# arancormonk/mbelib-neo

Measured on AMD Instinct MI355X. Metric: 20ms frames/sec (whole node) + PCM RMS error vs reference, IMBE 7200x4400, higher is better.
Workload: dtype f32

## Files before the change

mbelib-neo_amd/csrc/mbx_expand_imbe.h:

```cpp
#pragma once
#include "mbx_device.h"
#include "mbx_expand_ambe.h"
#ifndef MBX_FTS
#define MBX_FTS(i, v) do { } while (0)
#endif

namespace mbx {
namespace xp {

__device__ __forceinline__ uint32_t low_bits_x(uint32_t v, int n) { return v & ((1u << n) - 1u); }

__device__ __forceinline__ void expand_imbe_frame_rec(bool have, uint4 rec, float* row, uint32_t* words, float* gains, int sub,
                                                      const DeviceTables& tabs) {
    const mbx_tables* T = tabs.t;
    {
        uint4* z = reinterpret_cast<uint4*>(&words[8 * sub]);
        z[0] = make_uint4(0u, 0u, 0u, 0u);
        z[1] = make_uint4(0u, 0u, 0u, 0u);
    }
    int bad = 1, L = 0, K = 0;
    float w0 = 0.0f;
    if (have) {
        const uint32_t w[3] = {rec.x, rec.y, rec.z};
        int b0 = (int)(w[0] >> 26);
        b0 = (b0 << 1) | rbit(w, 85);
        b0 = (b0 << 1) | rbit(w, 86);
        if (b0 <= 207) {
            const uint2 q = tabs.d->imbe_b0[b0];
            w0 = __uint_as_float(q.x);
            L = (int)(q.y & 0xffu);
            K = (int)(q.y >> 8);
            bad = (L == 0) ? 1 : 0;
        }
    } else {
        rec = make_uint4(0u, 0u, 0u, 0u);
    }
    MBX_FTS(5, L);
    const int L9 = bad ? 0 : L - 9;
    const bool live = have && !bad;
    const bool block_lane = live && sub >= 1 && sub <= 6;
    const DerivedTables* D = tabs.d;
    uint32_t e[10];
    {
        const uint16_t* bo = reinterpret_cast<const uint16_t*>(&T->imbe_bo[L9][0][0]);
#pragma unroll
        for (int t = 0; t < 10; ++t) {
            const int idx = 10 * sub + t;
            e[t] = bo[idx < 79 ? idx : 78];
        }
    }
    const int blk = block_lane ? sub : 1;
    const uint32_t info = D->imbe_blk_info[L9][blk];
    const int g = (sub >= 2 && sub <= 6) ? sub - 2 : 0;
    const float nb = T->imbe_ba[L9][g][0], step = T->imbe_ba[L9][g][1];
    float ric[7];
#pragma unroll
    for (int m = 1; m <= 6; ++m) {
        ric[m] = T->imbe_ri_cos[m][blk];
    }
    float qstep[11];
    uint32_t bmw[3];
    {
        const uint32_t* bp = reinterpret_cast<const uint32_t*>(&D->imbe_blk_bm[L9][blk][0]);
        bmw[0] = bp[0];
        bmw[1] = bp[1];
        bmw[2] = bp[2];
#pragma unroll
        for (int k = 2; k <= 10; ++k) {
            qstep[k] = D->imbe_blk_step[L9][blk][k];
        }
    }
    const int ji_rows = (int)((info >> 16) & 0xffu);
    const float* rows = &D->imbe_len_rows[ji_rows <= 10 ? ji_rows : 10][0][0];
    float cosr[10];
#pragma unroll
    for (int k = 0; k < 10; ++k) {
        cosr[k] = rows[k];
    }
    MBX_FTS(6, cosr[0]);
    wave_lds_sync();
    {
        const int s0 = 10 * sub + 6;
        const uint32_t hi = s0 < 32 ? rec.x : (s0 < 64 ? rec.y : rec.z), lo = s0 < 32 ? rec.y : (s0 < 64 ? rec.z : 0u);
        uint32_t window = (uint32_t)(((((uint64_t)hi << 32) | lo) << (s0 & 31)) >> 54);
        window &= (sub == 7) ? ~1u : ~0u;
#pragma unroll
        for (int t = 0; t < 10; ++t) {
            const uint32_t m = e[t] & 0xffu, pos = e[t] >> 8;
            atomicOr(&words[m], ((window >> (9 - t)) & 1u) << pos);
        }
    }
    wave_lds_sync();
    MBX_FTS(7, e[0]);
    float b2v = 0.0f;
    if (live && sub == 1) {
        b2v = T->imbe_B2[low_bits_x(words[2], 6)];
    }
    if (block_lane) {
        float G = b2v;
        if (sub != 1) {
            const int inb = (int)nb;
            const int bm = (int)low_bits_x(words[sub + 1], inb);
            G = (step * ((float)bm - ldexpf(1.0f, inb - 1) + 0.5f));
        }
        gains[sub] = G;
    }
    wave_lds_sync();
    MBX_FTS(8, b2v);
    const uint32_t b1 = low_bits_x(words[1], 12);
    uint32_t band_lo = 0u, band_hi = 0u;
#pragma unroll
    for (int h = 0; h < 2; ++h) {
        const int k = sub + 8 * h;
        if (k < 12 && k < K && ((b1 >> (K - 1 - k)) & 1u)) {
            const unsigned long long m = 7ULL << (3 * k);
            band_lo |= (uint32_t)m;
            band_hi |= (uint32_t)(m >> 32);
        }
    }
    band_lo = sum8(band_lo);
    band_hi = sum8(band_hi);
    if (have) {
        if (sub == 0) {
            uint32_t vlo = 0, vhi = 0;
            if (!bad) {
                unsigned long long v = ((unsigned long long)band_hi << 32) | band_lo;
                if (b1 & 1u) {
                    v |= ~0ULL << (3 * K);
                }
                v &= (L >= 64) ? ~0ULL : ((1ULL << L) - 1ULL);
                vlo = (uint32_t)v;
                vhi = (uint32_t)(v >> 32);
            }
            row[0] = 0.0f;
            row[57] = __uint_as_float(vlo);
            row[58] = __uint_as_float(vhi);
            row[59] = w0;
            row[60] = __int_as_float(L);
            row[61] = __int_as_float(K);
            row[62] = __uint_as_float(rec.w);
            row[63] = __int_as_float(bad);
        } else if (block_lane) {
            const int m0 = (int)(info & 0xffu), l0 = (int)((info >> 8) & 0xffu), ji = (int)((info >> 16) & 0xffu);
            float C2[11];
            {
                float sum = 0;
#pragma unroll
                for (int m = 1; m <= 6; ++m) {
                    const float am = (m == 1) ? 1.0f : 2.0f;
                    sum = sum + (am * gains[m] * ric[m]);
                }
                C2[1] = sum;
            }
#pragma unroll
            for (int k = 2; k <= 10; ++k) {
                const int Bm = (int)((bmw[k >> 2] >> (8 * (k & 3))) & 0xffu);
                const int bm = (int)low_bits_x(words[m0 + k - 2], Bm);
                const float v = (qstep[k] * (((float)bm - ldexpf(1.0f, Bm - 1)) + 0.5f));
                C2[k] = 2.0f * v;
            }
            float next[10];
            auto fetch = [&](float (&dst)[10], int j) {
                const float* nr = rows + 10 * (j < ji ? j : ji - 1);
#pragma unroll
                for (int k = 0; k < 10; ++k) {
                    dst[k] = nr[k];
                }
            };
            auto output = [&](const float (&c)[10], int j) {
                float sum = 0;
#pragma unroll
                for (int k = 1; k <= 10; ++k) {
                    sum = sum + (C2[k] * c[k - 1]);
                }
                row[l0 + j - 1] = sum;
            };
            for (int j = 1; j <= ji; j += 2) {
                fetch(next, j);
                output(cosr, j);
                if (j + 1 <= ji) {
                    fetch(cosr, j + 1);
                    output(next, j + 1);
                }
            }
        }
    }
}

}
}
```

mbelib-neo_amd/csrc/mbx_stream.hip:

```cpp
#include <type_traits>

#include "mbx_device.h"
#include "mbx_kernels.h"
#include "mbx_expand_ambe.h"
#ifdef MBX_STAGE_TIMES
namespace mbx {
constexpr int kStageWaves = 65536;
__device__ unsigned g_stage_buf[kStageWaves * 16];
__shared__ unsigned long long s_stage_prev;
}
#define MBX_TS(i)                                                                          \
    do {                                                                                   \
        const unsigned long long t_ = wall_clock64();                                      \
        if ((threadIdx.x & 63) == 0) {                                                     \
            if ((i) > 0 && blockIdx.x < (unsigned)mbx::kStageWaves) {                      \
                mbx::g_stage_buf[blockIdx.x * 16u + (unsigned)(i)] = (unsigned)(t_ - mbx::s_stage_prev);   \
            }                                                                              \
            mbx::s_stage_prev = t_;                                                        \
        }                                                                                  \
    } while (0)
#else
#define MBX_TS(i) do { } while (0)
#endif
#if defined(MBX_STAGE_TIMES) && defined(MBX_STAGE_SUB)
#define MBX_TSX(i) MBX_TS(i)
#else
#define MBX_TSX(i) do { } while (0)
#endif
#ifdef MBX_FRAME_STAMPS
namespace mbx { __device__ unsigned long long g_frame_stamps[16]; }
#define MBX_FSTAMP(i) do { g_frame_stamps[i] = wall_clock64(); } while (0)
#endif
#ifdef MBX_STAGE_TIMES
#define MBX_FTS(i, v) do { asm volatile("" :: "v"(v)); MBX_TS(i); } while (0)
#else
#define MBX_FTS(i, v) do { } while (0)
#endif
#include "mbx_fec_frame.h"
#include "mbx_front_imbe.h"

#ifndef MBX_PRIO_BANK
#define MBX_PRIO_BANK 2
#endif
#ifndef MBX_PRIO_FFT
#define MBX_PRIO_FFT 1
#endif
#ifndef MBX_PRIO_FRONT_IMBE
#define MBX_PRIO_FRONT_IMBE 3
#endif
#ifndef MBX_PRIO_FRONT_BLOCK
#define MBX_PRIO_FRONT_BLOCK 3
#endif
#ifndef MBX_PARK_N
#define MBX_PARK_N 8
#endif
#ifndef MBX_STREAM_WAVES_PER_SIMD
#define MBX_STREAM_WAVES_PER_SIMD 7
#endif

namespace mbx {

struct Parms {
    float    w0;
    int      L, K;
    int      Vl;
    float    Ml, log2Ml, PHIl, PSIl;
    float    gamma;
    uint32_t tonePhase;
    int      swn;
    float    localEnergy;
    int      amplitudeThreshold;
    float    errorRate;
    int      errorCountTotal, errorCount4, repeatCount;
    float    mutingThreshold;
    float    uw[4];
    float    noiseSeed;
    float    ov[2];
};

__device__ __forceinline__ float uni(float x) { return __int_as_float(__builtin_amdgcn_readfirstlane(__float_as_int(x))); }
__device__ __forceinline__ int uni(int x) { return __builtin_amdgcn_readfirstlane(x); }
__device__ __forceinline__ uint32_t uni(uint32_t x) { return (uint32_t)__builtin_amdgcn_readfirstlane((int)x); }

enum : int {
    O_W0 = 0, O_L = 1, O_K = 2, O_VL = 3, O_ML = 60, O_LOG2ML = 117, O_PHI = 174, O_PSI = 231, O_GAMMA = 288,
    O_TONEPHASE = 289, O_SWN = 290, O_LOCALENERGY = 291, O_AMPTHR = 292, O_ERRORRATE = 293, O_ERRTOTAL = 294,
    O_ERR4 = 295, O_REPEAT = 296, O_MUTETHR = 297, O_UW = 298, O_NOISESEED = 554, O_OVERLAP = 555, PARMS_DWORDS = 651
};

enum : int {
    H_W0 = 0, H_L = 1, H_K = 2, H_GAMMA = 3, H_TONEPHASE = 4, H_SWN = 5, H_LOCALENERGY = 6, H_AMPTHR = 7, H_ERRORRATE = 8,
    H_ERRTOTAL = 9, H_ERR4 = 10, H_REPEAT = 11, H_MUTETHR = 12, H_NOISESEED = 13
};
__device__ __forceinline__ uint32_t load_header(const mbe_parms* __restrict__ p, int lane) {
    const int j = lane & 15;
    const int idx = (j < 3) ? j : ((j < 13) ? (O_GAMMA - H_GAMMA) + j : O_NOISESEED);
    static_assert(O_MUTETHR - O_GAMMA == H_MUTETHR - H_GAMMA, "fields 3..12 of the header are contiguous in mbe_parms");
    return reinterpret_cast<const uint32_t*>(p)[idx];
}
__device__ __forceinline__ int hdr_i(uint32_t h, int k) { return __builtin_amdgcn_readlane((int)h, k); }
__device__ __forceinline__ float hdr_f(uint32_t h, int k) { return __int_as_float(__builtin_amdgcn_readlane((int)h, k)); }

template <bool kFlat = false>
__device__ __forceinline__ void load_parms_arrays(Parms& r, const mbe_parms* __restrict__ p, int lane) {
    const float* f = reinterpret_cast<const float*>(p);
    const int* i = reinterpret_cast<const int*>(p);
    const bool band = lane < MBX_BAND_SLOTS;
    if constexpr (kFlat) {
        const int vl = i[O_VL + lane];
        const float ml = f[O_ML + lane], l2 = f[O_LOG2ML + lane], ph = f[O_PHI + lane], ps = f[O_PSI + lane];
#pragma unroll
        for (int j = 0; j < 4; ++j) {
            r.uw[j] = f[O_UW + lane + 64 * j];
        }
        r.ov[0] = f[O_OVERLAP + lane];
        const float o1 = f[O_OVERLAP + 64 + (lane & 31)];
        r.Vl = band ? vl : 0;
        r.Ml = band ? ml : 0.0f;
        r.log2Ml = band ? l2 : 0.0f;
        r.PHIl = band ? ph : 0.0f;
        r.PSIl = band ? ps : 0.0f;
        r.ov[1] = (lane < 32) ? o1 : 0.0f;
        return;
    }
    r.Vl = band ? i[O_VL + lane] : 0;
    r.Ml = band ? f[O_ML + lane] : 0.0f;
    r.log2Ml = band ? f[O_LOG2ML + lane] : 0.0f;
    r.PHIl = band ? f[O_PHI + lane] : 0.0f;
    r.PSIl = band ? f[O_PSI + lane] : 0.0f;
#pragma unroll
    for (int j = 0; j < 4; ++j) {
        r.uw[j] = f[O_UW + lane + 64 * j];
    }
    r.ov[0] = f[O_OVERLAP + lane];
    r.ov[1] = (lane < 32) ? f[O_OVERLAP + 64 + lane] : 0.0f;
}
__device__ __forceinline__ void set_parms_header(Parms& r, uint32_t h) {
    r.w0 = hdr_f(h, H_W0);
    r.L = hdr_i(h, H_L);
    r.K = hdr_i(h, H_K);
    r.gamma = hdr_f(h, H_GAMMA);
    r.tonePhase = (uint32_t)hdr_i(h, H_TONEPHASE);
    r.swn = hdr_i(h, H_SWN);
    r.localEnergy = hdr_f(h, H_LOCALENERGY);
    r.amplitudeThreshold = hdr_i(h, H_AMPTHR);
    r.errorRate = hdr_f(h, H_ERRORRATE);
    r.errorCountTotal = hdr_i(h, H_ERRTOTAL);
    r.errorCount4 = hdr_i(h, H_ERR4);
    r.repeatCount = hdr_i(h, H_REPEAT);
    r.mutingThreshold = hdr_f(h, H_MUTETHR);
    r.noiseSeed = hdr_f(h, H_NOISESEED);
}
template <bool kGather = false>
__device__ __forceinline__ void load_parms(Parms& r, const mbe_parms* __restrict__ p, int lane) {
    if constexpr (kGather) {
        const uint32_t h = load_header(p, lane);
        load_parms_arrays(r, p, lane);
        set_parms_header(r, h);
        return;
    }
    const float* f = reinterpret_cast<const float*>(p);
    const int* i = reinterpret_cast<const int*>(p);
    r.w0 = uni(f[O_W0]);
    r.L = uni(i[O_L]);
    r.K = uni(i[O_K]);
    load_parms_arrays(r, p, lane);
    r.gamma = uni(f[O_GAMMA]);
    r.tonePhase = (uint32_t)uni(i[O_TONEPHASE]);
    r.swn = uni(i[O_SWN]);
    r.localEnergy = uni(f[O_LOCALENERGY]);
    r.amplitudeThreshold = uni(i[O_AMPTHR]);
    r.errorRate = uni(f[O_ERRORRATE]);
    r.errorCountTotal = uni(i[O_ERRTOTAL]);
    r.errorCount4 = uni(i[O_ERR4]);
    r.repeatCount = uni(i[O_REPEAT]);
    r.mutingThreshold = uni(f[O_MUTETHR]);
    r.noiseSeed = uni(f[O_NOISESEED]);
}

__device__ __forceinline__ int write_lane(int v, int uniform_value, int k) {
    asm("v_writelane_b32 %0, %1, %2" : "+v"(v) : "s"(__builtin_amdgcn_readfirstlane(uniform_value)), "n"(k));
    return v;
}
template <bool kNt, class T>
__device__ __forceinline__ void st_state(T* p, T v) {
    if constexpr (kNt) {
        __builtin_nontemporal_store(v, p);
    } else {
        *p = v;
    }
}
enum UwSkip : int { kUwStoreAll = 0, kUwSkipUpper = 1, kUwSkipAll = 2 };
__device__ __forceinline__ bool uw_all_zero_bits(float a, float b, float c = 0.0f, float d = 0.0f) {
    const uint32_t bits = (__float_as_uint(a) | __float_as_uint(b)) | (__float_as_uint(c) | __float_as_uint(d));
    return __ballot(bits != 0u) == 0ULL;
}
template <bool kGather = false, bool kNt = kGather, bool kSilent = false>
__device__ __forceinline__ void store_parms(const Parms& r, mbe_parms* __restrict__ p, int lane, UwSkip uw_skip = kUwStoreAll) {
    float* f = reinterpret_cast<float*>(p);
    int* i = reinterpret_cast<int*>(p);
    if constexpr (kGather) {
        int h = 0;
        h = write_lane(h, __float_as_int(r.w0), H_W0);
        h = write_lane(h, r.L, H_L);
        h = write_lane(h, r.K, H_K);
        h = write_lane(h, __float_as_int(r.gamma), H_GAMMA);
        h = write_lane(h, (int)r.tonePhase, H_TONEPHASE);
        h = write_lane(h, r.swn, H_SWN);
        h = write_lane(h, __float_as_int(r.localEnergy), H_LOCALENERGY);
        h = write_lane(h, r.amplitudeThreshold, H_AMPTHR);
        h = write_lane(h, __float_as_int(r.errorRate), H_ERRORRATE);
        h = write_lane(h, r.errorCountTotal, H_ERRTOTAL);
        h = write_lane(h, r.errorCount4, H_ERR4);
        h = write_lane(h, r.repeatCount, H_REPEAT);
        h = write_lane(h, __float_as_int(r.mutingThreshold), H_MUTETHR);
        h = write_lane(h, __float_as_int(r.noiseSeed), H_NOISESEED);
        if (lane < 14) {
            const int idx = (lane < 3) ? lane : ((lane < 13) ? (O_GAMMA - H_GAMMA) + lane : O_NOISESEED);
            st_state<kNt>(&i[idx], (int)(h));
        }
    } else if (lane == 0) {
        st_state<kNt>(&f[O_W0], (float)(r.w0));
        st_state<kNt>(&i[O_L], (int)(r.L));
        st_state<kNt>(&i[O_K], (int)(r.K));
        st_state<kNt>(&f[O_GAMMA], (float)(r.gamma));
        st_state<kNt>(&i[O_TONEPHASE], (int)((int)r.tonePhase));
        st_state<kNt>(&i[O_SWN], (int)(r.swn));
        st_state<kNt>(&f[O_LOCALENERGY], (float)(r.localEnergy));
        st_state<kNt>(&i[O_AMPTHR], (int)(r.amplitudeThreshold));
        st_state<kNt>(&f[O_ERRORRATE], (float)(r.errorRate));
        st_state<kNt>(&i[O_ERRTOTAL], (int)(r.errorCountTotal));
        st_state<kNt>(&i[O_ERR4], (int)(r.errorCount4));
        st_state<kNt>(&i[O_REPEAT], (int)(r.repeatCount));
        st_state<kNt>(&f[O_MUTETHR], (float)(r.mutingThreshold));
        st_state<kNt>(&f[O_NOISESEED], (float)(r.noiseSeed));
    }
    if (lane < MBX_BAND_SLOTS) {
        st_state<kNt>(&i[O_VL + lane], (int)(r.Vl));
        st_state<kNt>(&f[O_ML + lane], (float)(r.Ml));
        st_state<kNt>(&f[O_LOG2ML + lane], (float)(r.log2Ml));
        st_state<kNt>(&f[O_PHI + lane], (float)(r.PHIl));
        st_state<kNt>(&f[O_PSI + lane], (float)(r.PSIl));
    }
    if constexpr (kSilent) {
        if (uw_skip != kUwSkipAll) {
            st_state<kNt>(&f[O_UW + lane], (float)(r.uw[0]));
            st_state<kNt>(&f[O_UW + lane + 64], (float)(r.uw[1]));
        }
        if (uw_skip == kUwStoreAll) {
            st_state<kNt>(&f[O_UW + lane + 128], (float)(r.uw[2]));
            st_state<kNt>(&f[O_UW + lane + 192], (float)(r.uw[3]));
        }
    } else {
#pragma unroll
        for (int j = 0; j < 4; ++j) {
            st_state<kNt>(&f[O_UW + lane + 64 * j], (float)(r.uw[j]));
        }
    }
    st_state<kNt>(&f[O_OVERLAP + lane], (float)(r.ov[0]));
    if (lane < 32) {
        st_state<kNt>(&f[O_OVERLAP + 64 + lane], (float)(r.ov[1]));
    }
}

template <bool kFlat = false>
__device__ __forceinline__ void load_prev_arrays(Parms& r, const mbe_parms* __restrict__ p, int lane) {
    const float* f = reinterpret_cast<const float*>(p);
    const bool band = lane < MBX_BAND_SLOTS;
    r = Parms{};
    if constexpr (kFlat) {
        const float ml = f[O_ML + lane], l2 = f[O_LOG2ML + lane], ph = f[O_PHI + lane];
        r.Ml = band ? ml : 0.0f;
        r.log2Ml = band ? l2 : 0.0f;
        r.PHIl = band ? ph : 0.0f;
        return;
    }
    r.Ml = band ? f[O_ML + lane] : 0.0f;
    r.log2Ml = band ? f[O_LOG2ML + lane] : 0.0f;
    r.PHIl = band ? f[O_PHI + lane] : 0.0f;
}
__device__ __forceinline__ void set_prev_header(Parms& r, uint32_t h) {
    r.L = hdr_i(h, H_L);
    r.gamma = hdr_f(h, H_GAMMA);
    r.errorRate = hdr_f(h, H_ERRORRATE);
    r.repeatCount = hdr_i(h, H_REPEAT);
    r.mutingThreshold = hdr_f(h, H_MUTETHR);
}
__device__ __forceinline__ void load_prev_view(Parms& r, const mbe_parms* __restrict__ p, int lane) {
    const uint32_t h = load_header(p, lane);
    load_prev_arrays(r, p, lane);
    set_prev_header(r, h);
}

__device__ __forceinline__ void load_prev_view_lds(Parms& r, const mbe_parms* __restrict__ p, int lane) {
    const float* f = reinterpret_cast<const float*>(p);
    const int* i = reinterpret_cast<const int*>(p);
    load_prev_arrays(r, p, lane);
    r.L = uni(i[O_L]);
    r.gamma = uni(f[O_GAMMA]);
    r.errorRate = uni(f[O_ERRORRATE]);
    r.repeatCount = uni(i[O_REPEAT]);
    r.mutingThreshold = uni(f[O_MUTETHR]);
}

template <bool kFlat = false>
__device__ __forceinline__ void load_enh_arrays(Parms& r, const mbe_parms* __restrict__ p, int lane) {
    const float* f = reinterpret_cast<const float*>(p);
    const int* i = reinterpret_cast<const int*>(p);
    const bool band = lane < MBX_BAND_SLOTS;
    r = Parms{};
    if constexpr (kFlat) {
        const int vl = i[O_VL + lane];
        const float ml = f[O_ML + lane], ph = f[O_PHI + lane], ps = f[O_PSI + lane];
        r.uw[2] = f[O_UW + lane + 128];
        r.uw[3] = f[O_UW + lane + 192];
        r.Vl = band ? vl : 0;
        r.Ml = band ? ml : 0.0f;
        r.PHIl = band ? ph : 0.0f;
        r.PSIl = band ? ps : 0.0f;
        return;
    }
    r.Vl = band ? i[O_VL + lane] : 0;
    r.Ml = band ? f[O_ML + lane] : 0.0f;
    r.PHIl = band ? f[O_PHI + lane] : 0.0f;
    r.PSIl = band ? f[O_PSI + lane] : 0.0f;
    r.uw[2] = f[O_UW + lane + 128];
    r.uw[3] = f[O_UW + lane + 192];
}
__device__ __forceinline__ void set_enh_header(Parms& r, uint32_t h) {
    r.w0 = hdr_f(h, H_W0);
    r.L = hdr_i(h, H_L);
    r.localEnergy = hdr_f(h, H_LOCALENERGY);
    r.amplitudeThreshold = hdr_i(h, H_AMPTHR);
}
__device__ __forceinline__ void load_enh_view(Parms& r, const mbe_parms* __restrict__ p, int lane) {
    const uint32_t h = load_header(p, lane);
    load_enh_arrays(r, p, lane);
    set_enh_header(r, h);
}

__device__ __forceinline__ void prev_header_of(Parms& r, const Parms& cur) {
    r.L = cur.L;
    r.gamma = cur.gamma;
    r.errorRate = cur.errorRate;
    r.repeatCount = cur.repeatCount;
    r.mutingThreshold = cur.mutingThreshold;
}
__device__ __forceinline__ void enh_view_of(Parms& r, const Parms& cur) {
    r = Parms{};
    r.Vl = cur.Vl;
    r.Ml = cur.Ml;
    r.PHIl = cur.PHIl;
    r.PSIl = cur.PSIl;
    r.uw[2] = cur.uw[2];
    r.uw[3] = cur.uw[3];
}

__device__ __forceinline__ void load_continuity(Parms& r, const mbe_parms* __restrict__ p, int lane) {
    const float* f = reinterpret_cast<const float*>(p);
    const bool band = lane < MBX_BAND_SLOTS;
    r.PHIl = band ? f[O_PHI + lane] : 0.0f;
    r.PSIl = band ? f[O_PSI + lane] : 0.0f;
#pragma unroll
    for (int j = 0; j < 4; ++j) {
        r.uw[j] = f[O_UW + lane + 64 * j];
    }
    r.noiseSeed = uni(f[O_NOISESEED]);
    r.ov[0] = f[O_OVERLAP + lane];
    r.ov[1] = (lane < 32) ? f[O_OVERLAP + 64 + lane] : 0.0f;
}

typedef float v2f __attribute__((ext_vector_type(2)));
__device__ __forceinline__ v2f splat(float x) { return v2f{x, x}; }

template <int kParkColsT>
struct WaveScratchT {
    static constexpr int kParkCols = kParkColsT;
    union {
        struct {
            alignas(16) float4 coef_amp[64];
            alignas(16) float4 coef_drift[64];
            alignas(16) float4 icoef[8];
        };
        struct {
            uint32_t words[64];
            float    gains[12];
            float    C[84];
            float    fp[64];
        } x;
        struct {
            float2 fft[256];
            float  bins[144];
        };
    };
    float park[kParkColsT > 0 ? kParkColsT : 1][kParkColsT > 0 ? 64 : 4];
};
using WaveScratch = WaveScratchT<MBX_PARK_N>;

constexpr uint32_t lcg_mul_steps(int n) {
    uint64_t a = 1;
    for (int k = 0; k < n; ++k) {
        a = (a * 171u) % 53125u;
    }
    return (uint32_t)a;
}
constexpr uint32_t lcg_add_steps(int n) {
    uint64_t c = 0;
    for (int k = 0; k < n; ++k) {
        c = (c * 171u + 11213u) % 53125u;
    }
    return (uint32_t)c;
}
constexpr int kDppWaveShr1 = 0x138;
__device__ __forceinline__ float seq_sum4(float v, int L, float* , int ) {
    float acc = v;
    const int n = uni(L);
    auto step = [&]() {
        const float below = __int_as_float(__builtin_amdgcn_update_dpp(0, __float_as_int(acc), kDppWaveShr1, 0xf, 0xf, true));
        acc = below + v;
    };
    int t = n - 1;
    for (; t >= 4; t -= 4) {
        step();
        step();
        step();
        step();
    }
    for (; t > 0; --t) {
        step();
    }
    return __int_as_float(__builtin_amdgcn_readlane(__float_as_int(acc), n & 63));
}

struct StreamRng {
    unsigned long long cn_seed48;
    uint32_t           cn_seeded, unv_state, unv_override;
};

typedef const __attribute__((address_space(4))) mbx_tables* ConstTables;
typedef const __attribute__((address_space(4))) DerivedTables* ConstDerived;
#define MBX_GLOBAL __attribute__((address_space(1)))
typedef const MBX_GLOBAL mbx_tables* GlobalTables;
typedef const MBX_GLOBAL DerivedTables* GlobalDerived;
typedef const MBX_GLOBAL float* GlobalFloats;
__device__ __forceinline__ uint32_t low_bits(uint32_t v, int n) { return v & ((1u << n) - 1u); }

template <class T>
__device__ __forceinline__ T tab_at(const void* uniform_base, size_t uniform_bytes, uint32_t lane_bytes) {
    const MBX_GLOBAL char* p = (const MBX_GLOBAL char*)uniform_base + uniform_bytes;
    asm("" : "+s"(p));
    return *(const MBX_GLOBAL T*)(p + lane_bytes);
}

__device__ __forceinline__ uint4 load_record_scalar(const mbx_param_record* rp) {
    const __attribute__((address_space(4))) uint32_t* rq = (const __attribute__((address_space(4))) uint32_t*)rp;
    return make_uint4(rq[0], rq[1], rq[2], rq[3]);
}

struct ImbeExpandReq {
    int      bad, L;
    uint32_t w0_bits, lk;
    uint32_t e0, e1, own;
    v2f      bas;
    float    b2, qs, sd;
    int      Bm;
// ... 417 lines not shown

__device__ __forceinline__ unsigned long long java_lcg_jump(unsigned long long s, int k) {
    const unsigned long long mask = (1ULL << 48) - 1ULL;
    unsigned long long A = 1, C = 0, a = 0x5DEECE66DULL, c = 0xBULL;
    for (int bit = 0; bit < 8; ++bit) {
        if ((k >> bit) & 1) {
            C = (a * C + c) & mask;
            A = (A * a) & mask;
        }
        c = (a * c + c) & mask;
        a = (a * a) & mask;
    }
    return (A * s + C) & mask;
}

__device__ void comfort_noise(float out[3], StreamRng& rng, int lane) {
    if (!rng.cn_seeded) {
        rng.cn_seed48 = (0x12345678ULL ^ 0x5DEECE66DULL) & ((1ULL << 48) - 1ULL);
        rng.cn_seeded = 1;
    }
    const float gain = (0.003f * 32767.0f) / 7.0f;
#pragma unroll
    for (int j = 0; j < 3; ++j) {
        const int n = lane + 64 * j;
        const unsigned long long s = java_lcg_jump(rng.cn_seed48, n + 1);
        const float u = ((float)(uint32_t)(s >> 24) / 16777216.0f) * 2.0f - 1.0f;
        out[j] = u * gain;
    }
    rng.cn_seed48 = java_lcg_jump(rng.cn_seed48, 160);
}

__device__ __forceinline__ v2f cmul_pk(v2f u, v2f w) {
    v2f t, d;
    asm("v_pk_mul_f32 %0, %1, %2 op_sel_hi:[0,1]" : "=v"(t) : "v"(u), "v"(w));
    asm("v_pk_fma_f32 %0, %1, %2, %3 op_sel:[1,1,0] op_sel_hi:[1,0,1] neg_lo:[0,1,0]" : "=v"(d) : "v"(u), "v"(w), "v"(t));
    return d;
}
__device__ __forceinline__ v2f cmul_cw(v2f u, v2f w) {
    v2f t, d;
    asm("v_pk_mul_f32 %0, %1, %2 op_sel_hi:[0,1] neg_hi:[0,1]" : "=v"(t) : "v"(u), "v"(w));
    asm("v_pk_fma_f32 %0, %1, %2, %3 op_sel:[1,1,0] op_sel_hi:[1,0,1]" : "=v"(d) : "v"(u), "v"(w), "v"(t));
    return d;
}
__device__ __forceinline__ v2f cmul_cu(v2f u, v2f w) {
    v2f t, d;
    asm("v_pk_mul_f32 %0, %1, %2 op_sel_hi:[0,1]" : "=v"(t) : "v"(u), "v"(w));
    asm("v_pk_fma_f32 %0, %1, %2, %3 op_sel:[1,1,0] op_sel_hi:[1,0,1] neg_hi:[0,1,0]" : "=v"(d) : "v"(u), "v"(w), "v"(t));
    return d;
}
__device__ __forceinline__ v2f add_mi(v2f a, v2f b) {
    v2f d;
    asm("v_pk_add_f32 %0, %1, %2 op_sel:[0,1] op_sel_hi:[1,0] neg_hi:[0,1]" : "=v"(d) : "v"(a), "v"(b));
    return d;
}
__device__ __forceinline__ v2f sub_mi(v2f a, v2f b) {
    v2f d;
    asm("v_pk_add_f32 %0, %1, %2 op_sel:[0,1] op_sel_hi:[1,0] neg_lo:[0,1]" : "=v"(d) : "v"(a), "v"(b));
    return d;
}

__device__ __forceinline__ float wrap_two_pi(float x, bool active) {
    const float y = 2.0f * (float)M_PI;
    if (__ballot(active && !(x >= 0.0f && x < 4.0e6f)) != 0ULL) {
        float w = fmodf(x, y);
        if (w < 0.0f) {
            w += y;
        }
        return w;
    }
    const float n = truncf(x * (0.15915494f * 1.000001f));
    float r = fmaf(-n, y, x);
    if (r < 0.0f) {
        r += y;
    }
    return r;
}

__device__ __forceinline__ float div_by_uniform(float a, float b, float rcp_b) {
    const float q = a * rcp_b;
    const float r = fmaf(-q, b, a);
    return fmaf(r, rcp_b, q);
}

template <bool kSnap, bool kPark = false, class Scratch = WaveScratch, bool kEarly = false, bool kDriftUnrolled = false>
__device__ bool synth_core(float out[3], Parms& cur, Parms& prev, bool have_rm0, float rm0, StreamRng& rng,
                           Scratch& S, const DeviceTables& tabs, int lane, const mbe_parms* snap_ptr = nullptr) {
    constexpr int kParkN = Scratch::kParkCols;
    if (kSnap && !kPark) {
        asm volatile("" : "+s"(snap_ptr));
    }
    const mbe_parms* const snap = kSnap ? snap_ptr : nullptr;
    auto snap_f = [&](int dword) -> float {
        if constexpr (kPark) {
            return reinterpret_cast<const float*>(snap)[dword];
        } else {
            return ((GlobalFloats)snap)[dword];
        }
    };
    GlobalDerived D = (GlobalDerived)tabs.d;
    constexpr int N = 160;
    out[0] = out[1] = out[2] = 0.0f;
    __builtin_amdgcn_s_setprio(0);
    if (cur.L < 1 || cur.L > 56 || prev.L < 1 || prev.L > 56) {
        return false;
    }
    if (!have_rm0) {
        const bool in = lane >= 1 && lane <= cur.L;
        rm0 = seq_sum4(in ? (cur.Ml * cur.Ml) : 0.0f, cur.L, reinterpret_cast<float*>(S.fft), lane);
    }
    smooth(cur, prev, rm0, lane, (kSnap && have_rm0) ? reinterpret_cast<const float*>(snap) + O_ML : nullptr,
           reinterpret_cast<float*>(S.fft));

    const bool rate_mutes = fabsf(cur.mutingThreshold - MBE_MUTING_THRESHOLD_AMBE) > 1e-6f;
    if (cur.repeatCount >= MBE_MAX_FRAME_REPEATS || (rate_mutes && cur.errorRate > cur.mutingThreshold)) {
        comfort_noise(out, rng, lane);
        return false;
    }

    float nz[4];
    const bool cold = cur.noiseSeed < 0.0f;
    const uint32_t x0 = cold ? 0u : (((uint32_t)cur.noiseSeed) % 53125u);
    auto lcg_req = [&](int k) -> uint32_t {
        k = k < 0 ? 0 : k;
        return tab_at<uint32_t>(tabs.d, offsetof(DerivedTables, lcg_pack), 4u * (uint32_t)k);
    };
    auto lcg_val = [&](uint32_t w) -> float {
        return (float)((__umul24(w & 0xffffu, x0) + (w >> 16)) % 53125u);
    };
    auto at = [&](int k) -> float { return lcg_val(lcg_req(k)); };
    constexpr uint32_t kMul160 = lcg_mul_steps(160), kAdd160 = lcg_add_steps(160);
    if (cold) {
        nz[0] = nz[1] = nz[2] = nz[3] = 0.0f;
        cur.ov[0] = cur.ov[1] = 0.0f;
        if (rng.unv_override) {
            cur.noiseSeed = uni((float)rng.unv_state);
            rng.unv_override = 0;
        } else {
            cur.noiseSeed = 3147.0f;
        }
    } else {
        nz[0] = cur.ov[0];
        if (!snap) {
            nz[1] = (lane < 32) ? cur.ov[1] : at(lane - 32);
            nz[2] = at(lane + 32);
            nz[3] = at(lane + 96);
            cur.ov[0] = at(lane + 64);
            cur.ov[1] = (lane < 32) ? at(lane + 128) : 0.0f;
        }
        cur.noiseSeed = (float)((kMul160 * x0 + kAdd160) % 53125u);
    }
    if (snap) {
        nz[1] = nz[2] = nz[3] = 0.0f;
        cur.ov[0] = cur.ov[1] = 0.0f;
    }

    MBX_TSX(14);
    int maxl;
    if (cur.L > prev.L) {
        maxl = cur.L;
        if (lane > prev.L && lane <= maxl) {
            prev.Ml = 0.0f;
            prev.Vl = 1;
        }
    } else {
        maxl = prev.L;
        if (lane > cur.L && lane <= maxl) {
            cur.Ml = 0.0f;
            cur.Vl = 1;
        }
    }

    const int numUv = popc64(__ballot(lane <= cur.L && cur.Vl == 0));
    const float cw0 = cur.w0, pw0 = prev.w0;
    const float inv_L = ((ConstDerived)tabs.d)->l_ratio[1][cur.L];
    if (lane >= 1 && lane <= 56 && !MBX_ABL(tabs, 64)) {
        float wrapped = wrap_two_pi(prev.PSIl, lane >= 1 && lane <= 56);
        prev.PSIl = wrapped;
        cur.PSIl = wrapped + ((pw0 + cw0) * ((float)(lane * N) / 2.0f));
        if (lane <= (cur.L / 4)) {
            cur.PHIl = cur.PSIl;
        } else {
            const float pl = ((2.0f * (float)M_PI / 53125.0f) * nz[0]) - (float)M_PI;
            cur.PHIl = cur.PSIl + div_by_uniform((float)numUv * pl, (float)cur.L, inv_L);
        }
    }

    uint32_t q64_early = 0u, q128_early = 0u;
    constexpr bool kEarlyNoise = kSnap && kEarly;
    if (kEarlyNoise && snap && !cold) {
        q64_early = lcg_req(lane + 64);
        q128_early = lcg_req(lane < 32 ? lane + 128 : 160);
        asm volatile("" ::: "memory");
    }

    MBX_TSX(15);
    const bool band = lane >= 1 && lane <= maxl;
    const bool cv = band && (cur.Vl == 1);
    const bool pv = band && (prev.Vl == 1);
    const bool stable = fabsf(cw0 - pw0) < (0.1f * cw0);
    const bool interp = (lane < 8) && cv && pv && stable;
    float acc[3] = {0.0f, 0.0f, 0.0f};

    unsigned long long imask = MBX_ABL(tabs, 16) ? 0ULL : __ballot(interp);
    if (imask) {
        if (lane < 8) {
            float4 k = make_float4(0.0f, 0.0f, 0.0f, 0.0f);
            if (interp) {
                const float dphi = cur.PHIl - prev.PHIl - (((pw0 + cw0) * (float)(lane * N)) / 2.0f);
                const float dw = (1.0f / (float)N)
                                 * (dphi - (2.0f * (float)M_PI * floorf((dphi + (float)M_PI) / (2.0f * (float)M_PI))));
                k = make_float4(prev.PHIl, (pw0 * (float)lane) + dw, 2.0f * prev.Ml, 2.0f * (cur.Ml - prev.Ml));
            }
            S.icoef[lane] = k;
        }
        wave_lds_sync();
        const float dw0 = cw0 - pw0;
        auto term = [&](auto flat, v2f phi, v2f a, v2f fl, v2f amp0, v2f damp, v2f nf, v2f nfrac) -> v2f {
            v2f theta = phi + (a * nf);
            if constexpr (!decltype(flat)::value) {
                v2f nq = nf;
                asm volatile("" : "+v"(nq));
                theta = theta + ((splat(dw0) * (fl * (nq * nq))) * splat(1.0f / 320.0f));
            }
            const v2f hi = theta * splat(0.15915494f);
            const v2f lo = __builtin_elementwise_fma(theta, splat(6.4206382e-9f),
                                                     __builtin_elementwise_fma(theta, splat(0.15915494f), -hi));
            const v2f r = v2f{__builtin_amdgcn_fractf(hi.x), __builtin_amdgcn_fractf(hi.y)} + lo;
            const v2f cs = {__builtin_amdgcn_cosf(r.x), __builtin_amdgcn_cosf(r.y)};
            return __builtin_elementwise_fma(nfrac, damp, amp0) * cs;
        };
        const float nf0 = (float)lane, nf2 = nf0 + 128.0f;
        const v2f nf01 = {nf0, nf0 + 64.0f};
        const v2f nfrac01 = {D->nfrac[lane], D->nfrac[lane + 64]};
        const float nfrac2 = D->nfrac[lane + 128];
        v2f acc01 = {0.0f, 0.0f}, acc2 = {0.0f, 0.0f};
        auto run = [&](auto flat) {
            while (imask) {
                const int la = __ffsll((long long)imask) - 1;
                imask &= imask - 1;
                const int lb = imask ? (__ffsll((long long)imask) - 1) : 0;
                imask &= imask - 1;
                const float4 ka = S.icoef[la], kb = S.icoef[lb];
                acc01 += term(flat, splat(ka.x), splat(ka.y), splat((float)la), splat(ka.z), splat(ka.w), nf01, nfrac01);
                if (lb) {
                    acc01 += term(flat, splat(kb.x), splat(kb.y), splat((float)lb), splat(kb.z), splat(kb.w), nf01, nfrac01);
                }
                acc2 += term(flat, v2f{ka.x, kb.x}, v2f{ka.y, kb.y}, v2f{(float)la, (float)lb}, v2f{ka.z, kb.z}, v2f{ka.w, kb.w},
                             splat(nf2), splat(nfrac2));
            }
        };
        if (dw0 == 0.0f) {
            run(std::true_type{});
        } else {
            run(std::false_type{});
        }
        acc[0] += acc01.x;
        acc[1] += acc01.y;
        if (lane < 32) {
            acc[2] += acc2.x + acc2.y;
        }
    }

    MBX_TSX(10);
    {
        const bool wv_p = pv && !interp && !MBX_ABL(tabs, 4), wv_c = cv && !interp && !MBX_ABL(tabs, 4);
        const bool any = (__ballot(wv_p || wv_c) != 0ULL) && !MBX_ABL(tabs, 8);
        if (any) {
            constexpr double kInv2Pi = 0.15915494309189533577;
            constexpr int kMidPrev = 52, kMidCur = 108;
            float drift_w;
            {
                const float fl = (float)lane;
                const float pw0l = pw0 * fl, cw0l = cw0 * fl;
                float4 ca = make_float4(0.0f, 0.0f, 0.0f, 0.0f), cd = ca;
                float c, d;
                unit_phasor_hw(fma((double)pw0l, (double)kMidPrev * kInv2Pi, (double)prev.PHIl * kInv2Pi), c, d);
                if (wv_p) {
                    const float g = 2.0f * prev.Ml, dl = -fmaf(pw0, fl, -pw0l);
                    const float A = g * c, B = g * d;
                    ca.x = A;
                    ca.z = B;
                    cd.x = dl * B;
                    cd.z = dl * A;
                }
                unit_phasor_hw(fma((double)cw0l, (double)kMidCur * kInv2Pi, (double)(cur.PHIl - (cw0l * (float)N)) * kInv2Pi), c, d);
                if (wv_c) {
                    const float g = 2.0f * cur.Ml, dl = -fmaf(cw0, fl, -cw0l);
                    const float A = g * c, B = g * d;
                    ca.y = A;
                    ca.w = B;
                    cd.y = dl * B;
                    cd.w = dl * A;
                }
                S.coef_amp[lane] = ca;
                S.coef_drift[lane] = cd;
                drift_w = (fabsf(cd.x) + fabsf(cd.z)) + (fabsf(cd.y) + fabsf(cd.w));
            }
            const bool need_drift = !(wave_sum(drift_w) * (float)(kMidPrev * 7) < 0.125f);
            v2f Ec, Es;
            {
                float c, d;
                unit_phasor(((double)pw0 * kInv2Pi) * (double)lane, c, d);
                Ec.x = c;
                Es.x = d;
                unit_phasor(((double)cw0 * kInv2Pi) * (double)lane, c, d);
                Ec.y = c;
                Es.y = d;
            }
            const int kk = lane <= kMidPrev ? lane : kMidPrev;
            auto Ws = [&](int i) -> float { return tab_at<float>(tabs.t, offsetof(mbx_tables, ws), 4u * (uint32_t)i); };
            const v2f w_plus = {Ws(N + kMidPrev + kk), Ws(kMidCur + (kk < 52 ? kk : 51))};
            const v2f w_minus = {Ws(N + kMidPrev - kk), Ws(kMidCur - kk)};
            wave_lds_sync();
            MBX_TS(5);
            __builtin_amdgcn_s_setprio(MBX_PRIO_BANK);
            v2f even = {0.0f, 0.0f}, odd = {0.0f, 0.0f}, even_d = {0.0f, 0.0f}, odd_d = {0.0f, 0.0f};
            const unsigned long long live = __ballot(wv_p || wv_c);
            const int last = 63 - __clzll((long long)live);
            const bool from8 = (live & 0xfeULL) == 0ULL;
// ... 723 lines not shown
        load_prev_arrays<kFlat>(prev_first, slot_prev, lane_in);
        load_parms_arrays<kFlat>(cur, slot_cur, lane_in);
        if constexpr (kRes) {
            asm volatile("" ::: "memory");
            if (!elided1) {
                h_prev_first = load_header(slot_prev, lane_in);
                h_enh_first = load_header(slot_enh, lane_in);
                load_enh_arrays<kFlat>(enh_first, slot_enh, lane_in);
            }
        } else {
            load_enh_arrays<kFlat>(enh_first, enh_src, lane_in);
        }
        mbx_param_record* const rec_out = const_cast<mbx_param_record*>(&records[fbase]);
        auto L_of = [&](int b0) -> int {
            return (b0 <= 207) ? (int)((__builtin_amdgcn_readlane((int)l_lanes, b0 & 63) >> (8 * (b0 >> 6))) & 0xff) : 0;
        };
        auto front_in_wave_7200 = [&]() {
            asm volatile("" : "+s"(frame_words.d[0]), "+s"(frame_words.d[1]), "+s"(frame_words.d[2]), "+s"(frame_words.d[3]),
                         "+s"(frame_words.d[4])::"memory");
            MBX_TS(14);
            const LaneFecHead head = lane_fec_imbe_head(frame_words, (reinterpret_cast<uintptr_t>(frame_ptr) & 2u) != 0u, lane_tabs, tabs_in.t,
                                                        lane_in);
            expand_imbe_request(xreq, head.b0, tabs_in.t, tabs_in.d, lane_in, L_of(head.b0));
            asm volatile("" ::: "memory");
            MBX_TS(15);
            rec_in = broadcast_record(lane_fec_imbe_tail(head, lane_tabs, hgen, tabs_in.t, lane_in), rec_out, lane_in);
            MBX_TS(10);
            expand_imbe_finish(rec_in, xreq, scratch, lane_in);
            MBX_TS(11);
        };
        if constexpr (kFuse == 3) {
            asm volatile("" ::: "memory");
            bool ready = uni(flag_v) == link.epoch;
            for (int tries = 0; !ready && tries < MBX_FRONT_SPIN; ++tries) {
                __builtin_amdgcn_s_sleep(8);
                ready = uni(__hip_atomic_load(link.flag, __ATOMIC_RELAXED, __HIP_MEMORY_SCOPE_AGENT)) == link.epoch;
            }
            if (ready) {
                const uint32_t* const rowp = reinterpret_cast<const uint32_t*>(&params[fbase].v[0]);
                row_first = __uint_as_float(__hip_atomic_load(rowp + lane_in, __ATOMIC_RELAXED, __HIP_MEMORY_SCOPE_AGENT));
                have_row = true;
            } else {
                frame_words = frame_fetch_scalar_imbe(frame_ptr);
                fetch_hgen();
                lane_tabs = lane_fec_request(tabs_in.d, lane_in);
                l_lanes = tab_at<uint32_t>(tabs_in.d, offsetof(DerivedTables, imbe_L_lanes), 4u * (uint32_t)lane_in);
                front_in_wave_7200();
                have_row = false;
                if (link.fallbacks && lane_in == 0) {
                    atomicAdd(link.fallbacks, 1u);
                }
            }
        } else if constexpr (kFuse != 0) {
            asm volatile("" ::: "memory");
            if constexpr (kFuse == 1) {
                front_in_wave_7200();
            } else {
                wire_in = frame_words_to_wire(frame_ptr, frame_words);
                const PrLane pr_lanes(lane_in);
                fused_tab.lanes = &pr_lanes;
#pragma unroll
                for (int k = 0; k < 9; ++k) {
                    wire_in.h[k] = uni(wire_in.h[k]);
                }
                rec_in = broadcast_record(fec_imbe7100x4400_wire(fused_tab, wire_in), rec_out, lane_in);
                const int b0 = imbe_record_b0(rec_in);
                expand_imbe_request(xreq, b0, tabs_in.t, tabs_in.d, lane_in, L_of(b0));
                MBX_TS(10);
                expand_imbe_finish(rec_in, xreq, scratch, lane_in);
                MBX_TS(11);
            }
        }
        set_parms_header(cur, h_cur);
        MBX_TS(1);
    } else {
        slot_prev = home_prev;
        slot_enh = home_enh;
        load_parms<kOne>(cur, slot_cur, lane_in);
        load_rng(rng, &rngs[slot]);
    }

    const int frames = (kOne && Tn > 1) ? 1 : Tn;
    UwSkip skip_cur = kUwStoreAll;
    for (int t = 0; t < frames; ++t) {
        const size_t f = fbase + (size_t)t;
        DeviceTables ft = tabs_in;
        int lane = lane_in;
        asm volatile("" : "+s"(ft.t), "+s"(ft.d), "+v"(lane));
        if constexpr (kPark) {
            lane &= 63;
        }
        const DeviceTables& tabs = ft;
        if constexpr (kPark && !kFrame) {
            __builtin_amdgcn_s_setprio(MBX_PRIO_FRONT_IMBE);
        }
        Parms enh;
        Parms prev;
        if constexpr (kPark) {
            enh = enh_keep;
            load_prev_view_lds(prev, slot_prev, lane);
        } else if constexpr (kOne) {
            prev = prev_first;
            if (kRes && elided1) {
                prev_header_of(prev, cur);
                enh_view_of(enh, cur);
                enh.w0 = cur.w0;
                enh.L = cur.L;
                enh.localEnergy = cur.localEnergy;
                enh.amplitudeThreshold = cur.amplitudeThreshold;
            } else {
                set_prev_header(prev, h_prev_first);
                enh = enh_first;
                set_enh_header(enh, h_enh_first);
            }
        } else {
            load_enh_view(enh, elided1 ? slot_cur : slot_enh, lane);
            load_prev_view(prev, slot_prev, lane);
        }
        if constexpr (kFuse == 3) {
            if (have_row) {
                scratch.x.fp[lane] = row_first;
                wave_lds_sync();
            }
        } else if (params) {
            scratch.x.fp[lane] = kOne ? row_first : params[f].v[lane];
            wave_lds_sync();
        } else if constexpr (kFuse != 0) {
        } else {
            expand_imbe_wave(kFrame ? rec_in : load_record_scalar(&records[f]), scratch, tabs.t, tabs.d, lane);
        }
        MBX_STAMP(3, false);
        if constexpr (kOne) { MBX_TS(2); }
        const float* fp = scratch.x.fp;
        const uint32_t errw = uni(__float_as_uint(fp[62]));
        const int c0 = (int)(errw & 0xffu), prot = (int)((errw >> 8) & 0xffu), c4 = (int)((errw >> 16) & 0xffu);
        unsigned flags = (errw >> 24) & 0xffu;
        const int total = c0 + prot;
        bool muted;
        bool cur_uw_was_zero = false, enh_uw_was_zero = false;
        {

            cur.errorCount4 = c4;
            cur.mutingThreshold = MBE_MUTING_THRESHOLD_IMBE;
            cur.errorCountTotal = total;
            cur.errorRate = uni((0.95f * prev.errorRate) + (0.000365f * (float)total));

            const int bad = MBX_ABL(tabs, 1) ? 0 : decode_imbe(fp, cur, prev, tabs.d, lane, scratch.x.C);
            if constexpr (kOne) {
                cur_uw_was_zero = uw_all_zero_bits(cur.uw[0], cur.uw[1], cur.uw[2], cur.uw[3]);
                enh_uw_was_zero = !kRes && uw_all_zero_bits(enh.uw[2], enh.uw[3]);
            }
            const float repeat_threshold = 10.0f + (40.0f * cur.errorRate);
            const bool c0_valid = (flags & MBE_PROCESS_FLAG_C0_VALID) != 0u;
            const bool repeat =
                (bad == 1) || (c0_valid ? ((c0 >= 2) && ((float)total >= repeat_threshold)) : (total > 5));
            if (!repeat) {
                cur.repeatCount = 0;
            } else {
                if (prev.repeatCount > (MBE_MAX_FRAME_REPEATS - 1)) {
                    imbe_headroom_reset(cur, lane);
                } else {
                    if (prev_partial) {
                        copy_parms<kOne>(slot_prev, home_prev, lane);
                        slot_fence<kPark>();
                    }
                    load_parms<kOne>(cur, slot_prev, lane);
                    cur.Ml = prev.Ml;
                    cur.log2Ml = prev.log2Ml;
                    cur.repeatCount++;
                }
                flags |= MBE_PROCESS_FLAG_REPEAT;
            }
            muted = (cur.repeatCount >= MBE_MAX_FRAME_REPEATS) || (cur.errorRate > cur.mutingThreshold);
        }
        MBX_STAMP(4, false);
        if constexpr (kOne) { MBX_TS(3); }
        if (!MBX_ABL(tabs, 256)) store_parms<kOne>(cur, slot_prev, lane);
        prev_partial = false;
        cur.log2Ml = 0.0f;
        cur.uw[0] = cur.uw[1] = cur.uw[2] = cur.uw[3] = 0.0f;
        float out[3] = {0.0f, 0.0f, 0.0f};
        bool fresh = false;
        {
            const float rm0 = MBX_ABL(tabs, 2) ? 1.0f : enhance(cur, lane, scratch.x.C);
            MBX_STAMP(5, false);
            if constexpr (kOne) { MBX_TS(4); }
            if (!MBX_ABL(tabs, 128)) {
                fresh = synth_core<true, kPark, ScratchT, kOne, kOne>(out, cur, enh, true, rm0, rng, scratch, tabs, lane, slot_prev);
            }
            MBX_STAMP(6, false);
            if constexpr (kOne) { MBX_TS(12); }
        }
        {
            slot_fence<kPark>();
            const float* f = reinterpret_cast<const float*>(slot_prev);
            if constexpr (!kPark) {
                asm volatile("" : "+s"(f));
            }
            if (lane < MBX_BAND_SLOTS) {
                cur.log2Ml = slot_read<kPark>(f, O_LOG2ML + lane);
            }
            if (!fresh) {
#pragma unroll
                for (int j = 0; j < 4; ++j) {
                    cur.uw[j] = slot_read<kPark>(f, O_UW + lane + 64 * j);
                }
                cur.ov[0] = slot_read<kPark>(f, O_OVERLAP + lane);
                cur.ov[1] = (lane < 32) ? slot_read<kPark>(f, O_OVERLAP + 64 + lane) : 0.0f;
            }
        }
        if (muted) {
            flags |= MBE_PROCESS_FLAG_MUTE;
        }
        UwSkip skip_enh = kUwStoreAll;
        if constexpr (kOne) {
            const bool uw_is_zero = uw_all_zero_bits(cur.uw[0], cur.uw[1], cur.uw[2], cur.uw[3]);
            skip_cur = (uw_is_zero && cur_uw_was_zero) ? kUwSkipAll : kUwStoreAll;
            skip_enh = (uw_is_zero && enh_uw_was_zero) ? kUwSkipUpper : kUwStoreAll;
        }
        if constexpr (kPark) {
            enh_keep = Parms{};
            enh_keep.w0 = cur.w0;
            enh_keep.L = cur.L;
            enh_keep.Vl = cur.Vl;
            enh_keep.Ml = cur.Ml;
            enh_keep.PHIl = cur.PHIl;
            enh_keep.PSIl = cur.PSIl;
            enh_keep.localEnergy = cur.localEnergy;
            enh_keep.amplitudeThreshold = cur.amplitudeThreshold;
            enh_keep.uw[2] = cur.uw[2];
            enh_keep.uw[3] = cur.uw[3];
        } else if (res1) {
            if (lane == 0) {
                res1[slot] = 1u;
            }
        } else {
            if (!MBX_ABL(tabs, 512)) store_parms<kOne, kOne, kOne>(cur, slot_enh, lane, skip_enh);
        }
        if (t + 1 < Tn) {
            slot_fence<kPark>();
        }

        store_pcm(out, f, pcm16, pcmf, lane);
        if (results && lane == 0) {
            mbe_process_result r;
            r.c0_errors = c0;
            r.protected_errors = total - c0;
            r.c4_errors = c4;
            r.total_errors = total;
            r.flags = flags;
            results[f] = r;
        }
    }

    if (!MBX_ABL(tabs_in, 1024)) store_parms<kOne, kOne, kOne>(cur, slot_cur, lane_in, skip_cur);
    store_rng(rng, &rngs[slot], lane_in);
    if constexpr (kPark) {
        if (res) {
            if (Tn > 0 && lane_in == 0) {
                res[slot] = 1u;
            }
        } else {
            store_parms<kOne>(cur, home_enh, lane_in);
        }
        wave_lds_sync();
        if (!prev_partial) {
            copy_parms<kOne>(home_prev, slot_prev, lane_in);
        }
        if constexpr (kFrame) {
            if (shadow.state) {
                store_parms<kOne, false>(cur, &shadow.state[0], lane_in);
                store_parms<kOne, false>(cur, &shadow.state[2], lane_in);
                copy_parms(&shadow.state[1], slot_prev, lane_in);
                store_rng(rng, shadow.rng, lane_in);
                if (lane_in == 0) {
                    *shadow.ok = 1u;
                }
            }
        }
    }
    MBX_STAMP(7, false);
    if constexpr (kOne) { MBX_TS(13); }
    MBX_STAMP(8, true);
}

__device__ __forceinline__ void front_block_imbe(int chunk, int S, const uint8_t* __restrict__ frames, mbx_param_record* __restrict__ records,
                                                 FrameParams* __restrict__ rows, uint32_t* __restrict__ flags, uint32_t epoch,
                                                 const DeviceTables& tabs, void* lds) {
    constexpr int kRowPad = 65;
    float (*tile)[kRowPad] = reinterpret_cast<float (*)[kRowPad]>(lds);
    uint32_t (*words)[64] = reinterpret_cast<uint32_t (*)[64]>(reinterpret_cast<char*>(lds) + 8 * kRowPad * 4);
    float (*gains)[8] = reinterpret_cast<float (*)[8]>(reinterpret_cast<char*>(lds) + 8 * kRowPad * 4 + 8 * 64 * 4);
    const int lane = lane_id();
    const int fi = lane >> 3, sub = lane & 7;
    const int j = 8 * chunk + fi;
    const bool have = j < S;
    MBX_TS(0);
    __builtin_amdgcn_s_setprio(MBX_PRIO_FRONT_BLOCK);
    const int sj = have ? (tabs.reverse ? (S - 1 - j) : j) : 0;
    const uint4 rec = front8_fec_imbe(have, frames + 18u * (size_t)sj, tabs, lane);
    if (have && sub == 0) {
        *reinterpret_cast<uint4*>(&records[sj]) = rec;
    }
    xp::expand_imbe_frame_rec(have, rec, tile[fi], words[fi], gains[fi], sub, tabs);
    wave_lds_sync();
    MBX_TS(9);
#pragma unroll
    for (int q = 0; q < 8; ++q) {
        const int jq = 8 * chunk + q;
        if (jq < S) {
            const int sq = tabs.reverse ? (S - 1 - jq) : jq;
            __hip_atomic_store(reinterpret_cast<uint32_t*>(&rows[sq].v[0]) + lane, __float_as_uint(tile[q][lane]), __ATOMIC_RELAXED,
                               __HIP_MEMORY_SCOPE_AGENT);
        }
    }
    asm volatile("s_waitcnt vmcnt(0)" ::: "memory");
    MBX_TS(10);
    if (lane == 0) {
        __hip_atomic_store(&flags[chunk], epoch, __ATOMIC_RELAXED, __HIP_MEMORY_SCOPE_AGENT);
    }
}

template <bool kRes>
__device__ __forceinline__ void imbe_one_launch_body(int S, int lead, const uint8_t* __restrict__ frames, mbx_param_record* __restrict__ records,
                                                     FrameParams* __restrict__ rows, uint32_t* __restrict__ flags, uint32_t* __restrict__ fallbacks,
                                                     uint32_t epoch, mbe_parms* __restrict__ state, mbx_stream_rng* __restrict__ rngs, int16_t* __restrict__ pcm16,
                                                     float* __restrict__ pcmf, mbe_process_result* __restrict__ results, const DeviceTables& tabs_in) {
    const int C = (S + 7) >> 3;
    const int D = lead < C ? (lead < 0 ? 0 : lead) : C;
    const int G = C - D;
    const int bid = (int)blockIdx.x;
    int chunk = -1, pos = -1;
    if (bid < D) {
        chunk = bid;
    } else {
        const int q = bid - D;
        if (q < 9 * G) {
            const int g = q / 9, r = q - 9 * g;
// ... 1336 lines not shown
```

Before: 346.2 million.

## Compact interpolation coefficients into packed pairs in LDS for vectorized synthesis

Adds a pair-packed LDS layout for the per-harmonic interpolation coefficients. Active lanes compact their records by popcount slot, and the synthesis loop walks the pairs with vector loads and two-wide terms instead of a per-bit ffs loop. This path is enabled by default for the single-frame variant. Two other changes, packed DCT multiplies and a shared precomputed header for parameter stores, sit behind macros that default to off. The compaction adds popcount work and a differently ordered accumulation, which may slightly change floating-point results.

```diff
diff --git a/mbelib-neo_amd/csrc/mbx_expand_imbe.h b/mbelib-neo_amd/csrc/mbx_expand_imbe.h
--- a/mbelib-neo_amd/csrc/mbx_expand_imbe.h
+++ b/mbelib-neo_amd/csrc/mbx_expand_imbe.h
@@ -5,11 +5,18 @@
 #define MBX_FTS(i, v) do { } while (0)
 #endif
 
+#ifndef MBX_TRIM_DCT_PACKED
+#define MBX_TRIM_DCT_PACKED 0
+#endif
+
 namespace mbx {
 namespace xp {
 
+typedef float f2 __attribute__((ext_vector_type(2)));
+
 __device__ __forceinline__ uint32_t low_bits_x(uint32_t v, int n) { return v & ((1u << n) - 1u); }
 
+template <bool kPackedDct = (MBX_TRIM_DCT_PACKED != 0)>
 __device__ __forceinline__ void expand_imbe_frame_rec(bool have, uint4 rec, float* row, uint32_t* words, float* gains, int sub,
                                                       const DeviceTables& tabs) {
     const mbx_tables* T = tabs.t;
@@ -169,9 +176,18 @@
             };
             auto output = [&](const float (&c)[10], int j) {
                 float sum = 0;
-#pragma unroll
-                for (int k = 1; k <= 10; ++k) {
-                    sum = sum + (C2[k] * c[k - 1]);
+                if constexpr (kPackedDct) {
+#pragma unroll
+                    for (int k = 1; k <= 10; k += 2) {
+                        const f2 p = f2{C2[k], C2[k + 1]} * f2{c[k - 1], c[k]};
+                        sum = sum + p.x;
+                        sum = sum + p.y;
+                    }
+                } else {
+#pragma unroll
+                    for (int k = 1; k <= 10; ++k) {
+                        sum = sum + (C2[k] * c[k - 1]);
+                    }
                 }
                 row[l0 + j - 1] = sum;
             };
diff --git a/mbelib-neo_amd/csrc/mbx_stream.hip b/mbelib-neo_amd/csrc/mbx_stream.hip
--- a/mbelib-neo_amd/csrc/mbx_stream.hip
+++ b/mbelib-neo_amd/csrc/mbx_stream.hip
@@ -54,6 +54,12 @@
 #ifndef MBX_PARK_N
 #define MBX_PARK_N 8
 #endif
+#ifndef MBX_TRIM_ICOEF_PAIRS
+#define MBX_TRIM_ICOEF_PAIRS 1
+#endif
+#ifndef MBX_TRIM_SHARED_HEADER
+#define MBX_TRIM_SHARED_HEADER 0
+#endif
 #ifndef MBX_STREAM_WAVES_PER_SIMD
 #define MBX_STREAM_WAVES_PER_SIMD 7
 #endif
@@ -195,26 +201,31 @@
     const uint32_t bits = (__float_as_uint(a) | __float_as_uint(b)) | (__float_as_uint(c) | __float_as_uint(d));
     return __ballot(bits != 0u) == 0ULL;
 }
-template <bool kGather = false, bool kNt = kGather, bool kSilent = false>
-__device__ __forceinline__ void store_parms(const Parms& r, mbe_parms* __restrict__ p, int lane, UwSkip uw_skip = kUwStoreAll) {
+__device__ __forceinline__ int gather_header(const Parms& r) {
+    int h = 0;
+    h = write_lane(h, __float_as_int(r.w0), H_W0);
+    h = write_lane(h, r.L, H_L);
+    h = write_lane(h, r.K, H_K);
+    h = write_lane(h, __float_as_int(r.gamma), H_GAMMA);
+    h = write_lane(h, (int)r.tonePhase, H_TONEPHASE);
+    h = write_lane(h, r.swn, H_SWN);
+    h = write_lane(h, __float_as_int(r.localEnergy), H_LOCALENERGY);
+    h = write_lane(h, r.amplitudeThreshold, H_AMPTHR);
+    h = write_lane(h, __float_as_int(r.errorRate), H_ERRORRATE);
+    h = write_lane(h, r.errorCountTotal, H_ERRTOTAL);
+    h = write_lane(h, r.errorCount4, H_ERR4);
+    h = write_lane(h, r.repeatCount, H_REPEAT);
+    h = write_lane(h, __float_as_int(r.mutingThreshold), H_MUTETHR);
+    h = write_lane(h, __float_as_int(r.noiseSeed), H_NOISESEED);
+    return h;
+}
+template <bool kGather = false, bool kNt = kGather, bool kSilent = false, bool kHeader = false>
+__device__ __forceinline__ void store_parms(const Parms& r, mbe_parms* __restrict__ p, int lane, UwSkip uw_skip = kUwStoreAll,
+                                            int header = 0) {
     float* f = reinterpret_cast<float*>(p);
     int* i = reinterpret_cast<int*>(p);
     if constexpr (kGather) {
-        int h = 0;
-        h = write_lane(h, __float_as_int(r.w0), H_W0);
-        h = write_lane(h, r.L, H_L);
-        h = write_lane(h, r.K, H_K);
-        h = write_lane(h, __float_as_int(r.gamma), H_GAMMA);
-        h = write_lane(h, (int)r.tonePhase, H_TONEPHASE);
-        h = write_lane(h, r.swn, H_SWN);
-        h = write_lane(h, __float_as_int(r.localEnergy), H_LOCALENERGY);
-        h = write_lane(h, r.amplitudeThreshold, H_AMPTHR);
-        h = write_lane(h, __float_as_int(r.errorRate), H_ERRORRATE);
-        h = write_lane(h, r.errorCountTotal, H_ERRTOTAL);
-        h = write_lane(h, r.errorCount4, H_ERR4);
-        h = write_lane(h, r.repeatCount, H_REPEAT);
-        h = write_lane(h, __float_as_int(r.mutingThreshold), H_MUTETHR);
-        h = write_lane(h, __float_as_int(r.noiseSeed), H_NOISESEED);
+        const int h = kHeader ? header : gather_header(r);
         if (lane < 14) {
             const int idx = (lane < 3) ? lane : ((lane < 13) ? (O_GAMMA - H_GAMMA) + lane : O_NOISESEED);
             st_state<kNt>(&i[idx], (int)(h));
@@ -372,6 +383,8 @@
 
 typedef float v2f __attribute__((ext_vector_type(2)));
 __device__ __forceinline__ v2f splat(float x) { return v2f{x, x}; }
+typedef float v4f __attribute__((ext_vector_type(4)));
+constexpr int kIPairFloats = 12;
 
 template <int kParkColsT>
 struct WaveScratchT {
@@ -380,7 +393,10 @@
         struct {
             alignas(16) float4 coef_amp[64];
             alignas(16) float4 coef_drift[64];
-            alignas(16) float4 icoef[8];
+            union {
+                alignas(16) float4 icoef[8];
+                alignas(16) float ipair[4 * kIPairFloats];
+            };
         };
         struct {
             uint32_t words[64];
@@ -964,7 +980,8 @@
     return fmaf(r, rcp_b, q);
 }
 
-template <bool kSnap, bool kPark = false, class Scratch = WaveScratch, bool kEarly = false, bool kDriftUnrolled = false>
+template <bool kSnap, bool kPark = false, class Scratch = WaveScratch, bool kEarly = false, bool kDriftUnrolled = false,
+          bool kPairs = false>
 __device__ bool synth_core(float out[3], Parms& cur, Parms& prev, bool have_rm0, float rm0, StreamRng& rng,
                            Scratch& S, const DeviceTables& tabs, int lane, const mbe_parms* snap_ptr = nullptr) {
     constexpr int kParkN = Scratch::kParkCols;
@@ -1093,7 +1110,20 @@
                                  * (dphi - (2.0f * (float)M_PI * floorf((dphi + (float)M_PI) / (2.0f * (float)M_PI))));
                 k = make_float4(prev.PHIl, (pw0 * (float)lane) + dw, 2.0f * prev.Ml, 2.0f * (cur.Ml - prev.Ml));
             }
-            S.icoef[lane] = k;
+            if constexpr (kPairs) {
+                const uint32_t im = (uint32_t)imask;
+                const int slot = __popc(interp ? (im & ((1u << lane) - 1u)) : im);
+                if (interp || lane == 0) {
+                    float* rec = &S.ipair[kIPairFloats * (slot >> 1) + (slot & 1)];
+                    rec[0] = k.x;
+                    rec[2] = k.y;
+                    rec[4] = k.z;
+                    rec[6] = k.w;
+                    rec[8] = (float)lane;
+                }
+            } else {
+                S.icoef[lane] = k;
+            }
         }
         wave_lds_sync();
         const float dw0 = cw0 - pw0;
@@ -1117,6 +1147,21 @@
         const float nfrac2 = D->nfrac[lane + 128];
         v2f acc01 = {0.0f, 0.0f}, acc2 = {0.0f, 0.0f};
         auto run = [&](auto flat) {
+            if constexpr (kPairs) {
+                const int n = popc64(imask);
+                for (int s = 0; s < n; s += 2) {
+                    const float* rec = &S.ipair[kIPairFloats * (s >> 1)];
+                    const v4f pa = *reinterpret_cast<const v4f*>(rec), am = *reinterpret_cast<const v4f*>(rec + 4);
+                    const v2f fl = *reinterpret_cast<const v2f*>(rec + 8);
+                    const v2f phi = {pa.x, pa.y}, a = {pa.z, pa.w}, amp0 = {am.x, am.y}, damp = {am.z, am.w};
+                    acc01 += term(flat, splat(phi.x), splat(a.x), splat(fl.x), splat(amp0.x), splat(damp.x), nf01, nfrac01);
+                    if (s + 1 < n) {
+                        acc01 += term(flat, splat(phi.y), splat(a.y), splat(fl.y), splat(amp0.y), splat(damp.y), nf01, nfrac01);
+                    }
+                    acc2 += term(flat, phi, a, fl, amp0, damp, splat(nf2), splat(nfrac2));
+                }
+                return;
+            }
             while (imask) {
                 const int la = __ffsll((long long)imask) - 1;
                 imask &= imask - 1;
@@ -2006,6 +2051,11 @@
 
     const int frames = (kOne && Tn > 1) ? 1 : Tn;
     UwSkip skip_cur = kUwStoreAll;
+    constexpr bool kShareHeader = kOne && MBX_TRIM_SHARED_HEADER;
+    int header = 0;
+    bool header_made = false;
+    (void)header;
+    (void)header_made;
     for (int t = 0; t < frames; ++t) {
         const size_t f = fbase + (size_t)t;
         DeviceTables ft = tabs_in;
@@ -2110,7 +2160,8 @@
             MBX_STAMP(5, false);
             if constexpr (kOne) { MBX_TS(4); }
             if (!MBX_ABL(tabs, 128)) {
-                fresh = synth_core<true, kPark, ScratchT, kOne, kOne>(out, cur, enh, true, rm0, rng, scratch, tabs, lane, slot_prev);
+                fresh = synth_core<true, kPark, ScratchT, kOne, kOne, kOne && MBX_TRIM_ICOEF_PAIRS>(out, cur, enh, true, rm0, rng, scratch,
+                                                                                                    tabs, lane, slot_prev);
             }
             MBX_STAMP(6, false);
             if constexpr (kOne) { MBX_TS(12); }
@@ -2159,7 +2210,15 @@
                 res1[slot] = 1u;
             }
         } else {
-            if (!MBX_ABL(tabs, 512)) store_parms<kOne, kOne, kOne>(cur, slot_enh, lane, skip_enh);
+            if (!MBX_ABL(tabs, 512)) {
+                if constexpr (kShareHeader) {
+                    header = gather_header(cur);
+                    header_made = true;
+                    store_parms<kOne, kOne, kOne, true>(cur, slot_enh, lane, skip_enh, header);
+                } else {
+                    store_parms<kOne, kOne, kOne>(cur, slot_enh, lane, skip_enh);
+                }
+            }
         }
         if (t + 1 < Tn) {
             slot_fence<kPark>();
@@ -2177,7 +2236,16 @@
         }
     }
 
-    if (!MBX_ABL(tabs_in, 1024)) store_parms<kOne, kOne, kOne>(cur, slot_cur, lane_in, skip_cur);
+    if (!MBX_ABL(tabs_in, 1024)) {
+        if constexpr (kShareHeader) {
+            if (!header_made) {
+                header = gather_header(cur);
+            }
+            store_parms<kOne, kOne, kOne, true>(cur, slot_cur, lane_in, skip_cur, header);
+        } else {
+            store_parms<kOne, kOne, kOne>(cur, slot_cur, lane_in, skip_cur);
+        }
+    }
     store_rng(rng, &rngs[slot], lane_in);
     if constexpr (kPark) {
         if (res) {
```

Result: no change. 344.5 million (-0.5%).
